# vliu15/3d-brain-tumor-segmentation

Measured on AMD Instinct MI355X. Metric: training volumes/sec (2ch x 128^3), higher is better.
Workload: dtype f32; 1 GPU; BASELINE configs[1]: 2ch x 128^3, batch 1 per GPU, fp32, full fwd+bwd with Dice+KL+L2 VAE loss + Dice metric + TF-form Adam; CLI-default model (base_filters=32, depth=4, groups=8, reduction=8; 42,174,773 params); parallelism=dp1, global_batch=1

## Files before the change

### 3d-brain-tumor-segmentation_amd/csrc/block_bwd.hip

```cpp
#include "common.h"
#include "bts_internal.h"
#include "finalize_parts.h"

__global__ __launch_bounds__(256) void blk_bwd_reduce_kernel(const float* __restrict__ x, const float* __restrict__ dy,
                                                             const float* __restrict__ res, const float* __restrict__ sp,
                                                             const float* __restrict__ gamma, const float* __restrict__ beta,
                                                             const float* __restrict__ mean, const float* __restrict__ rstd,
                                                             double* partial, double* se_partial, float* __restrict__ ds_out, long E, long L,
                                                             long span, int C, int G, int cg, int lddy) {
  __shared__ double sh[256 * 8];
  const int unit = blockIdx.y, n = unit / G, gs = unit % G;
  const long unitBase = (long)gs * L;
  const long lo = (long)blockIdx.x * span;
  long hi = lo + span;
  if (hi > L) hi = L;
  const int F4 = C >> 2;
  const int cph = (int)((unitBase + lo + threadIdx.x * 4) % C);
  float gam[4], bet[4];
#pragma unroll
  for (int e = 0; e < 4; ++e) {
    const int idx = gs * cg + ((cph + e) % cg);
    gam[e] = gamma[idx];
    bet[e] = beta[idx];
  }
  const float m_s = mean[unit], rs_s = rstd[unit];
  double a[4] = {0, 0, 0, 0}, b[4] = {0, 0, 0, 0}, pa[4] = {0, 0, 0, 0}, pb[4] = {0, 0, 0, 0};
  const float* xb = x + (long)n * E + unitBase;
  const float* rb = res + (long)n * E + unitBase;
  const long pix0 = ((long)n * E + unitBase + lo + threadIdx.x * 4) / C;
  const long pstep = 1024 / C;
  const bool head = (threadIdx.x & (F4 - 1)) == 0;
  auto one = [&](const f32x4 v, const f32x4 r, const f32x4 d, float s, long pix) {
    float t = (d[0] * r[0] + d[1] * r[1]) + (d[2] * r[2] + d[3] * r[3]);
    for (int o = F4 >> 1; o > 0; o >>= 1) t += __shfl_xor(t, o, 64);
    const float dsv = t * s * (1.f - s);
    if (head) ds_out[pix] = dsv;
#pragma unroll
    for (int e = 0; e < 4; ++e) {
      const float xh = (v[e] - m_s) * rs_s;
      float de = d[e];
      if (!(xh * gam[e] + bet[e] > 0.f)) de = 0.f;
      a[e] += (double)(de * xh);
      b[e] += (double)de;
      pa[e] += (double)(d[e] * r[e]);
      pb[e] += (double)(dsv * r[e]);
    }
  };
  const long K = (hi - lo) / 1024;
  const long i0 = lo + threadIdx.x * 4;
  long k = 0;
  for (; k + 2 <= K; k += 2) {
    f32x4 v[2], r[2], d[2];
    float s[2];
#pragma unroll
    for (int u = 0; u < 2; ++u) {
      const long i = i0 + (k + u) * 1024, pix = pix0 + (k + u) * pstep;
      v[u] = *reinterpret_cast<const f32x4*>(xb + i);
      r[u] = *reinterpret_cast<const f32x4*>(rb + i);
      d[u] = *reinterpret_cast<const f32x4*>(dy + pix * lddy + cph);
      s[u] = sp[pix];
    }
#pragma unroll
    for (int u = 0; u < 2; ++u) one(v[u], r[u], d[u], s[u], pix0 + (k + u) * pstep);
  }
  for (; k < K; ++k) {
    const long i = i0 + k * 1024, pix = pix0 + k * pstep;
    one(*reinterpret_cast<const f32x4*>(xb + i), *reinterpret_cast<const f32x4*>(rb + i), *reinterpret_cast<const f32x4*>(dy + pix * lddy + cph), sp[pix],
        pix);
  }
#pragma unroll
  for (int e = 0; e < 4; ++e) { sh[threadIdx.x * 8 + e] = a[e]; sh[threadIdx.x * 8 + 4 + e] = b[e]; }
  __syncthreads();
  for (int j = threadIdx.x; j < cg; j += 256) {
    double sa = 0.0, sb = 0.0;
    if (cg >= 4) {
      const int e = j & 3, rr = j >> 2, P4 = cg >> 2;
      for (int q = rr; q < 256; q += P4) { sa += sh[q * 8 + e]; sb += sh[q * 8 + 4 + e]; }
    } else {
      for (int q = 0; q < 256; ++q)
        for (int e = j; e < 4; e += cg) { sa += sh[q * 8 + e]; sb += sh[q * 8 + 4 + e]; }
    }
    const long o = (((long)unit * gridDim.x + blockIdx.x) * cg + j) * 2;
    partial[o] = sa;
    partial[o + 1] = sb;
  }
  __syncthreads();
#pragma unroll
  for (int e = 0; e < 4; ++e) { sh[threadIdx.x * 8 + e] = pa[e]; sh[threadIdx.x * 8 + 4 + e] = pb[e]; }
  __syncthreads();
  const int vpb = 256 / F4;
  for (int col = threadIdx.x; col < C; col += 256) {
    const int e = col & 3, l = col >> 2;
    double sa = 0.0, sb = 0.0;
    for (int q = 0; q < vpb; ++q) { sa += sh[(q * F4 + l) * 8 + e]; sb += sh[(q * F4 + l) * 8 + 4 + e]; }
    const long o = ((((long)n * G + gs) * gridDim.x + blockIdx.x) * C + col) * 2;
    se_partial[o] = sa;
    se_partial[o + 1] = sb;
  }
}

__global__ __launch_bounds__(256) void blk_bwd_apply_kernel(const float* __restrict__ x, const float* __restrict__ dy, float* __restrict__ dx,
                                                            float* __restrict__ dres, const float* __restrict__ gamma,
                                                            const float* __restrict__ beta, const float* __restrict__ mean,
                                                            const float* __restrict__ rstd, const float* __restrict__ c1,
                                                            const float* __restrict__ c2, const float* __restrict__ sp,
                                                            const float* __restrict__ ds, const float* __restrict__ ch,
                                                            const float* __restrict__ wsp, const float* __restrict__ dgap, long chunks_per_unit,
                                                            int cpb, int C, int cg, int G, int lddy) {
  const long chunk0 = (long)blockIdx.x * cpb;
  const long unit = chunk0 / chunks_per_unit;
  const int g = (int)(unit % G), n = (int)(unit / G);
  const float m = mean[unit], rs = rstd[unit], k1 = c1[unit], k2 = c2[unit];
  const int c = (threadIdx.x * 4) % C;
  float ga[4], be[4];
#pragma unroll
  for (int e = 0; e < 4; ++e) {
    const int idx = g * cg + ((c + e) % cg);
    ga[e] = gamma[idx];
    be[e] = beta[idx];
  }
  const f32x4 chv = *reinterpret_cast<const f32x4*>(ch + (long)n * C + c);
  const f32x4 wsv = {wsp[c], wsp[c + 1], wsp[c + 2], wsp[c + 3]};
  const f32x4 dgv = *reinterpret_cast<const f32x4*>(dgap + (long)n * C + c);
  const long off = chunk0 * 1024 + threadIdx.x * 4;
  const long vpc = 1024 / C;
  const long pix = chunk0 * vpc + (threadIdx.x * 4) / C;
  const long doff = pix * lddy + c;
  const long dstep = vpc * lddy;
  auto one = [&](const f32x4 v, const f32x4 d, float s, float dsv, long o_) {
    f32x4 o, q;
#pragma unroll
    for (int e = 0; e < 4; ++e) {
      const float xh = (v[e] - m) * rs;
      float de = d[e];
      if (!(xh * ga[e] + be[e] > 0.f)) de = 0.f;
      o[e] = (de * ga[e] - k1 - xh * k2) * rs;
      q[e] = d[e] * (s + chv[e]) + dsv * wsv[e] + dgv[e];
    }
    *reinterpret_cast<f32x4*>(dx + o_) = o;
    *reinterpret_cast<f32x4*>(dres + o_) = q;
  };
  int k = 0;
  for (; k + 1 < cpb; k += 2) {
    const f32x4 v0 = *reinterpret_cast<const f32x4*>(x + off + (long)k * 1024);
    const f32x4 d0 = *reinterpret_cast<const f32x4*>(dy + doff + (long)k * dstep);
    const f32x4 v1 = *reinterpret_cast<const f32x4*>(x + off + (long)(k + 1) * 1024);
    const f32x4 d1 = *reinterpret_cast<const f32x4*>(dy + doff + (long)(k + 1) * dstep);
    const float s0 = sp[pix + (long)k * vpc], s1 = sp[pix + (long)(k + 1) * vpc];
    const float t0 = ds[pix + (long)k * vpc], t1 = ds[pix + (long)(k + 1) * vpc];
    one(v0, d0, s0, t0, off + (long)k * 1024);
    one(v1, d1, s1, t1, off + (long)(k + 1) * 1024);
  }
  for (; k < cpb; ++k) {
    const f32x4 v0 = *reinterpret_cast<const f32x4*>(x + off + (long)k * 1024);
    const f32x4 d0 = *reinterpret_cast<const f32x4*>(dy + doff + (long)k * dstep);
    one(v0, d0, sp[pix + (long)k * vpc], ds[pix + (long)k * vpc], off + (long)k * 1024);
  }
}

__global__ __launch_bounds__(256) void blk_bwd_middle_kernel(const double* partial, const float* gamma, float* dgamma, float* dbeta, float* c1,
                                                             float* c2, const double* se_partial, double* red, int N, int G, int B, int cg,
                                                             double L, int accum, int F) {
  __shared__ double sh[256 * 2];
  if ((int)blockIdx.x < G) gn_bwd_finalize_slab_body(partial, gamma, dgamma, dbeta, c1, c2, N, G, B, cg, L, accum, blockIdx.x, sh);
  else se_bwd_partial_reduce_body(se_partial, red, N, G * B, F, (int)blockIdx.x - G);
}

static bool blk_bwd_plan(int N, long V, int F, int R, int G, int* B, long* span) {
  if (N <= 0 || V <= 0 || R <= 0 || G <= 0 || F < 4 || F > 256 || (F & (F - 1)) != 0 || F % G != 0) return false;
  const long E = V * F;
  if (E % G != 0) return false;
  const long L = E / G;
  const int cg = F / G;
  if (L % 1024 != 0 || 1024 % F != 0 || 256 % cg != 0) return false;
  if (!bts_gn_slab_blocks_(N, V, F, G, B, span)) return false;
  return (long)N * G * (L / 1024) <= 0x7fffffffL;
}
extern "C" long bts_block_bwd_workspace(int N, long V, int F, int R, int G) {
  int B;
  long span;
  if (!blk_bwd_plan(N, V, F, R, G, &B, &span)) return -1;
  const int cg = F / G;
  return (long)N * G * B * cg * 2 * 8 + (long)N * G * 2 * 4 + 64
         + (long)N * G * B * F * 2 * 8 + ((long)N * F * 3 + (long)N * R) * 8 + 128;
}
extern "C" int bts_block_bwd(const float* dout, int lddo, const float* res, const float* c2x, const float* sp, const float* gap, const float* h,
                             const float* ch, const float* w1, const float* w2, const float* wsp, const float* gamma, const float* beta,
                             const float* mean, const float* rstd, float* dres, float* dc2, float* ds, float* dgap, float* dw1, float* dw2,
                             float* dwsp, float* dgamma, float* dbeta, void* workspace, long workspace_bytes, int N, long V, int F, int R, int G,
                             int accumulate_gate_params, int accumulate_norm_params, hipStream_t stream) {
  int B;
  long span;
  if (!blk_bwd_plan(N, V, F, R, G, &B, &span)) return BTS_ERR_UNSUPPORTED;
  if (lddo < F || lddo % 4 != 0) return BTS_ERR_ALIGN;
  if ((((uintptr_t)dout) & 15) || (((uintptr_t)res) & 15) || (((uintptr_t)c2x) & 15) || (((uintptr_t)dres) & 15) || (((uintptr_t)dc2) & 15) ||
      (((uintptr_t)ch) & 15) || (((uintptr_t)dgap) & 15))
    return BTS_ERR_ALIGN;
  if (workspace == nullptr || (((uintptr_t)workspace) & 15) || workspace_bytes < bts_block_bwd_workspace(N, V, F, R, G)) return BTS_ERR_WORKSPACE;
  const long E = V * F, L = E / G;
  const int cg = F / G;
  double* partial = reinterpret_cast<double*>(workspace);
  float* c1 = reinterpret_cast<float*>(partial + (long)N * G * B * cg * 2);
  float* c2 = c1 + (long)N * G;
  double* sep = reinterpret_cast<double*>((reinterpret_cast<uintptr_t>(c2 + (long)N * G) + 63) & ~(uintptr_t)63);
  double* red = sep + (long)N * G * B * F * 2;
  double* scratch = red + (long)N * F * 2;
  (void)hipGetLastError();
  hipLaunchKernelGGL(blk_bwd_reduce_kernel, dim3(B, N * G), dim3(256), 0, stream, c2x, dout, res, sp, gamma, beta, mean, rstd, partial, sep, ds, E, L,
                     span, F, G, cg, lddo);
  BTS_LAUNCH_CHECK();
  hipLaunchKernelGGL(blk_bwd_middle_kernel, dim3(G + (N * F + 3) / 4), dim3(256), 0, stream, partial, gamma, dgamma, dbeta, c1, c2, sep, red, N, G, B, cg,
                     (double)L, accumulate_norm_params, F);
  BTS_LAUNCH_CHECK();
  const int r = bts_se_mlp_bwd_(red, scratch, gap, h, ch, w1, w2, dw1, dw2, dwsp, dgap, N, G * B, V, F, R, accumulate_gate_params, stream);
  if (r != BTS_OK) return r;
  const long cpu = L / 1024;
  int cpb = 8;
  while (cpb > 1 && cpu % cpb != 0) cpb >>= 1;
  const long nblk = (long)N * G * cpu / cpb;
  hipLaunchKernelGGL(blk_bwd_apply_kernel, dim3((unsigned)nblk), dim3(256), 0, stream, c2x, dout, dc2, dres, gamma, beta, mean, rstd, c1, c2, sp, ds, ch,
                     wsp, dgap, cpu, cpb, F, cg, G, lddo);
  BTS_LAUNCH_CHECK();
  return BTS_OK;
}
```

### 3d-brain-tumor-segmentation_amd/csrc/finalize_parts.h

```cpp
#pragma once
#include "common.h"

__device__ __forceinline__ void gn_bwd_finalize_slab_body(const double* partial, const float* gamma, float* dgamma, float* dbeta, float* c1,
                                                          float* c2, int N, int G, int B, int cg, double L, int accum, int g, double* sh) {
  const int j = threadIdx.x % cg, sl = threadIdx.x / cg, S = 256 / cg;
  double ga = 0.0, gb = 0.0;
  for (int n = 0; n < N; ++n) {
    const long unit = (long)n * G + g;
    double sa = 0.0, sb = 0.0;
    for (int b = sl; b < B; b += S) {
      const double* o = partial + ((unit * B + b) * cg + j) * 2;
      sa += o[0]; sb += o[1];
    }
    __syncthreads();
    sh[threadIdx.x * 2] = sa; sh[threadIdx.x * 2 + 1] = sb;
    __syncthreads();
    if (sl == 0) {
      sa = 0.0; sb = 0.0;
      for (int s2 = 0; s2 < S; ++s2) { sa += sh[(s2 * cg + j) * 2]; sb += sh[(s2 * cg + j) * 2 + 1]; }
      ga += sa; gb += sb;
    }
    __syncthreads();
    if (sl == 0) {
      sh[j * 2] = (double)gamma[g * cg + j] * sb;
      sh[j * 2 + 1] = (double)gamma[g * cg + j] * sa;
    }
    __syncthreads();
    if (threadIdx.x == 0) {
      double s1 = 0.0, s2 = 0.0;
      for (int q = 0; q < cg; ++q) { s1 += sh[q * 2]; s2 += sh[q * 2 + 1]; }
      c1[unit] = (float)(s1 / L);
      c2[unit] = (float)(s2 / L);
    }
  }
  if (sl == 0) {
    const int idx = g * cg + j;
    if (dgamma) dgamma[idx] = accum ? dgamma[idx] + (float)ga : (float)ga;
    if (dbeta) dbeta[idx] = accum ? dbeta[idx] + (float)gb : (float)gb;
  }
}

__device__ __forceinline__ void se_bwd_partial_reduce_body(const double* partial, double* red, int N, int B, int F, int blk) {
  const int lane = threadIdx.x & 63;
  const int i = blk * 4 + (threadIdx.x >> 6);
  if (i >= N * F) return;
  const int n = i / F, c = i % F;
  double a = 0.0, b = 0.0;
  const double2* pp = reinterpret_cast<const double2*>(partial) + (long)n * B * F + c;
  int k = lane;
  for (; k + 7 * 64 < B; k += 8 * 64) {
    double2 v[8];
#pragma unroll
    for (int u = 0; u < 8; ++u) v[u] = pp[(long)(k + u * 64) * F];
#pragma unroll
    for (int u = 0; u < 8; ++u) { a += v[u].x; b += v[u].y; }
  }
  for (; k < B; k += 64) {
    const double2 v = pp[(long)k * F];
    a += v.x;
    b += v.y;
  }
  a = wave_sum_f64(a);
  b = wave_sum_f64(b);
  if (lane == 0) { red[i * 2] = a; red[i * 2 + 1] = b; }
}

__device__ __forceinline__ void se_mlp_bwd_param_body(const double* red, const float* gap, const float* hbuf, float* dw1, float* dw2, float* dwsp,
                                                      const double* scratch, int N, int F, int R, int accum, int blk) {
  const double* dz2 = scratch;
  const double* dz1 = scratch + (long)N * F;
  const int i = blk * 256 + threadIdx.x;
  if (i < R * F) {
    {
      const int k = i / F, c = i % F;
      double s = 0.0;
      for (int n = 0; n < N; ++n) s += (double)hbuf[n * R + k] * dz2[n * F + c];
      dw2[i] = accum ? dw2[i] + (float)s : (float)s;
    }
    {
      const int c = i / R, k = i % R;
      double s = 0.0;
      for (int n = 0; n < N; ++n) s += (double)gap[n * F + c] * dz1[n * R + k];
      dw1[i] = accum ? dw1[i] + (float)s : (float)s;
    }
  }
  if (i < F) {
    double s = 0.0;
    for (int n = 0; n < N; ++n) s += red[((long)n * F + i) * 2 + 1];
    dwsp[i] = accum ? dwsp[i] + (float)s : (float)s;
  }
}

__device__ __forceinline__ void lp_dbias_block(const float (&cs)[8], int oct, int noct, double* part_row, float* sh ) {
  __syncthreads();
#pragma unroll
  for (int e = 0; e < 8; ++e) sh[threadIdx.x * 8 + e] = cs[e];
  __syncthreads();
  if ((int)threadIdx.x < noct * 8) {
    const int o = threadIdx.x >> 3, e = threadIdx.x & 7;
    double s = 0.0;
    for (int t = o; t < 256; t += noct) s += (double)sh[t * 8 + e];
    part_row[o * 8 + e] = s;
  }
  (void)oct;
}
__device__ __forceinline__ void lp_dbias_finalize_body(const double* part, float* db, int nblocks, int C, int accum, int c, double* sh) {
  double s = 0.0;
  for (int b = threadIdx.x; b < nblocks; b += 256) s += part[(long)b * C + c];
  s = block_sum_f64(s, sh);
  if (threadIdx.x == 0) db[c] = accum ? db[c] + (float)s : (float)s;
}

__device__ __forceinline__ void lp_gn_bwd_finalize_body(const double* partial, const float* gamma, float* dgamma, float* dbeta, float* c1,
                                                        float* c2, int N, int G, int B, int cg, double L, int accum, int g, double* sh,
                                                        double* tot ) {
  const int t = threadIdx.x;
  int Np = 1;
  while (Np * 2 <= N && cg * Np * 2 <= 256) Np *= 2;
  const int S = 256 / (cg * Np);
  const int j = t % cg, nl = (t / cg) % Np, sl = t / (cg * Np);
  double ga = 0.0, gb = 0.0;
  for (int n0 = 0; n0 < N; n0 += Np) {
    const int n = n0 + nl;
    double sa = 0.0, sb = 0.0;
    if (n < N) {
      const long unit = (long)n * G + g;
      for (int b = sl; b < B; b += S) {
        const double* o = partial + ((unit * B + b) * cg + j) * 2;
        sa += o[0]; sb += o[1];
      }
    }
    __syncthreads();
    sh[t * 2] = sa; sh[t * 2 + 1] = sb;
    __syncthreads();
    if (sl == 0) {
      sa = 0.0; sb = 0.0;
      for (int s2 = 0; s2 < S; ++s2) { sa += sh[((s2 * Np + nl) * cg + j) * 2]; sb += sh[((s2 * Np + nl) * cg + j) * 2 + 1]; }
      tot[(nl * cg + j) * 2] = sa; tot[(nl * cg + j) * 2 + 1] = sb;
    }
    __syncthreads();
    if (t < Np && n0 + t < N) {
      double s1 = 0.0, s2 = 0.0;
      for (int q = 0; q < cg; ++q) {
        s1 += (double)gamma[g * cg + q] * tot[(t * cg + q) * 2 + 1];
        s2 += (double)gamma[g * cg + q] * tot[(t * cg + q) * 2];
      }
      const long unit = (long)(n0 + t) * G + g;
      c1[unit] = (float)(s1 / L);
      c2[unit] = (float)(s2 / L);
    }
    if (t < cg) {
      for (int q = 0; q < Np && n0 + q < N; ++q) { ga += tot[(q * cg + t) * 2]; gb += tot[(q * cg + t) * 2 + 1]; }
    }
  }
// ... 7 lines not shown
```

### 3d-brain-tumor-segmentation_amd/csrc/groupnorm.hip

```cpp
#include <stdlib.h>
#include "common.h"
#include "bts_internal.h"
#include "finalize_parts.h"

#define GN_BLOCKS_MAX 256

struct GnGeom {
  int N, C, G, cg, mode;
  long V;
  long E;
  long L;
  int B;
  long span;
  int generic;
};

static int gn_geom(GnGeom& g, int N, long V, int C, int G, int mode) {
  if (N <= 0 || V <= 0 || C <= 0 || G <= 0) return BTS_ERR_SHAPE;
  if (C < G || C % G != 0) return BTS_ERR_SHAPE;
  g.N = N; g.C = C; g.G = G; g.cg = C / G; g.mode = mode; g.V = V; g.E = V * C; g.L = g.E / G;
  if (g.E % G != 0) return BTS_ERR_UNSUPPORTED;
  g.generic = (C % 4 != 0 || (C & (C - 1)) != 0 || C > 1024 || g.L % 4 != 0) ? 1 : 0;
  const long unit = (mode == BTS_GN_SLAB) ? g.L : g.E;
  const int units = (mode == BTS_GN_SLAB) ? N * G : N;
// ... 238 lines not shown
  const int lane = threadIdx.x & 63, w = threadIdx.x >> 6;
  if (lane == 0) { sh[w] = s; sh[16 + w] = ss; }
  __syncthreads();
  if (threadIdx.x == 0) {
    double rs = 0.0, rss = 0.0;
    for (int k = 0; k < 16; ++k) { rs += sh[k]; rss += sh[16 + k]; }
    const double m = rs / count;
    double var = rss / count - m * m;
    if (var < 0.0) var = 0.0;
    mean[i] = (float)m;
    rstd[i] = (float)(1.0 / sqrt(var + (double)eps));
  }
}

int bts_gn_finalize_partials_(const double* partial, float* mean, float* rstd, int NG, long B, double count, float eps,
                              hipStream_t stream) {
  if (NG <= 0 || B <= 0 || B > 0x7fffffffL) return BTS_ERR_SHAPE;
  if (B >= 512) {
    if (((uintptr_t)partial) & 15) return BTS_ERR_ALIGN;
    (void)hipGetLastError(); hipLaunchKernelGGL(gn_stats_finalize_wide_kernel, dim3(NG), dim3(1024), 0, stream, partial, mean, rstd, (int)B, count, eps);
    BTS_LAUNCH_CHECK();
    return BTS_OK;
  }
  (void)hipGetLastError(); hipLaunchKernelGGL(gn_stats_finalize_kernel, dim3((NG + 3) / 4), dim3(256), 0, stream, partial, mean, rstd, NG, (int)B, 0,
                     1, BTS_GN_SLAB, count, eps);
  BTS_LAUNCH_CHECK();
  return BTS_OK;
}

__global__ __launch_bounds__(256) void gn_apply_kernel(const float* __restrict__ x, float* __restrict__ y,
                                                       const float* __restrict__ gamma, const float* __restrict__ beta,
                                                       const float* __restrict__ mean, const float* __restrict__ rstd,
                                                       long total4, long E, long L, int C, int G, int cg, int ldy,
                                                       int mode, int relu) {
  for (long f = blockIdx.x * (long)blockDim.x + threadIdx.x; f < total4; f += (long)gridDim.x * blockDim.x) {
    const long i = f * 4;
    const long n = i / E;
    const long r = i - n * E;
    const int c = (int)(r % C);
    const long pix = i / C;
    const f32x4 v = *reinterpret_cast<const f32x4*>(x + i);
    f32x4 o;
    if (mode == BTS_GN_SLAB) {
      const int g = (int)(r / L);
      const float m = mean[n * G + g], rs = rstd[n * G + g];
#pragma unroll
      for (int e = 0; e < 4; ++e) {
        const int idx = g * cg + ((c + e) % cg);
        o[e] = (v[e] - m) * rs * gamma[idx] + beta[idx];
      }
    } else {
#pragma unroll
      for (int e = 0; e < 4; ++e) {
        const int g = (c + e) / cg;
        o[e] = (v[e] - mean[n * G + g]) * rstd[n * G + g] * gamma[c + e] + beta[c + e];
      }
    }
    if (relu) {
#pragma unroll
      for (int e = 0; e < 4; ++e) o[e] = fmaxf(o[e], 0.f);
    }
    *reinterpret_cast<f32x4*>(y + pix * ldy + c) = o;
  }
}

__global__ __launch_bounds__(256) void gn_apply_slab_stream_kernel(const float* __restrict__ x, float* __restrict__ y,
                                                                   const float* __restrict__ gamma, const float* __restrict__ beta,
                                                                   const float* __restrict__ mean, const float* __restrict__ rstd,
                                                                   long chunks_per_unit, int cpb, int C, int cg, int G, int relu, int ldy) {
  const long chunk0 = (long)blockIdx.x * cpb;
  const long unit = chunk0 / chunks_per_unit;
  const int g = (int)(unit % G);
  const float m = mean[unit], rs = rstd[unit];
  const int c = (threadIdx.x * 4) % C;
  float sc[4], sh[4];
#pragma unroll
  for (int e = 0; e < 4; ++e) {
    const int idx = g * cg + ((c + e) % cg);
    sc[e] = rs * gamma[idx];
    sh[e] = beta[idx];
  }
  const float* xp = x + chunk0 * 1024 + threadIdx.x * 4;
  const long vpc = 1024 / C;
  float* yp = y + (chunk0 * vpc + (threadIdx.x * 4) / C) * ldy + c;
  const long ystep = vpc * ldy;
  int k = 0;
  for (; k + 1 < cpb; k += 2) {
    const f32x4 v0 = *reinterpret_cast<const f32x4*>(xp + (long)k * 1024);
    const f32x4 v1 = *reinterpret_cast<const f32x4*>(xp + (long)(k + 1) * 1024);
    f32x4 o0, o1;
#pragma unroll
    for (int e = 0; e < 4; ++e) {
      o0[e] = fmaf(v0[e] - m, sc[e], sh[e]);
      o1[e] = fmaf(v1[e] - m, sc[e], sh[e]);
      if (relu) { o0[e] = fmaxf(o0[e], 0.f); o1[e] = fmaxf(o1[e], 0.f); }
    }
    *reinterpret_cast<f32x4*>(yp + (long)k * ystep) = o0;
    *reinterpret_cast<f32x4*>(yp + (long)(k + 1) * ystep) = o1;
  }
  for (; k < cpb; ++k) {
    const f32x4 v0 = *reinterpret_cast<const f32x4*>(xp + (long)k * 1024);
    f32x4 o0;
#pragma unroll
    for (int e = 0; e < 4; ++e) {
      o0[e] = fmaf(v0[e] - m, sc[e], sh[e]);
      if (relu) o0[e] = fmaxf(o0[e], 0.f);
    }
    *reinterpret_cast<f32x4*>(yp + (long)k * ystep) = o0;
  }
}
static int gn_stream_cpb(long chunks_per_unit) {
  int cpb = 8;
  while (cpb > 1 && chunks_per_unit % cpb != 0) cpb >>= 1;
  return cpb;
}

extern "C" int bts_gn_apply(const float* x, float* y, const float* gamma, const float* beta, const float* mean,
                            const float* rstd, int N, long V, int C, int ldy, int G, int mode, int relu,
                            hipStream_t stream) {
  GnGeom g;
  int r = gn_geom(g, N, V, C, G, mode);
  if (r != BTS_OK) return r;
  if (g.generic || ldy % 4 != 0) {
    if (ldy < C) return BTS_ERR_ALIGN;
    const long total = (long)N * g.E;
    int gb = (int)((total + 255) / 256);
    if (gb > 8192) gb = 8192;
    (void)hipGetLastError(); hipLaunchKernelGGL(gn_apply_generic_kernel, dim3(gb), dim3(256), 0, stream, x, y, gamma, beta, mean, rstd, total, g.E, g.L,
                       C, G, g.cg, ldy, mode, relu);
    BTS_LAUNCH_CHECK();
    return BTS_OK;
  }
  if (ldy < C || (((uintptr_t)x) & 15) || (((uintptr_t)y) & 15)) return BTS_ERR_ALIGN;
  if (mode == BTS_GN_SLAB && g.L % 1024 == 0 && 1024 % C == 0) {
    const long cpu = g.L / 1024;
    const int cpb = gn_stream_cpb(cpu);
    const long nblk = (long)N * G * cpu / cpb;
    if (nblk <= 0x7fffffffL) {
      (void)hipGetLastError(); hipLaunchKernelGGL(gn_apply_slab_stream_kernel, dim3((unsigned)nblk), dim3(256), 0, stream, x, y, gamma, beta, mean,
                         rstd, cpu, cpb, C, g.cg, G, relu, ldy);
      BTS_LAUNCH_CHECK();
      return BTS_OK;
    }
  }
  const long total4 = (long)N * g.E / 4;
  int blocks = (int)((total4 + 255) / 256);
  if (blocks > 8192) blocks = 8192;
  (void)hipGetLastError(); hipLaunchKernelGGL(gn_apply_kernel, dim3(blocks), dim3(256), 0, stream, x, y, gamma, beta, mean, rstd, total4, g.E,
                     g.L, C, G, g.cg, ldy, mode, relu);
  BTS_LAUNCH_CHECK();
  return BTS_OK;
}

__global__ __launch_bounds__(256) void gn_bwd_reduce_kernel(const float* __restrict__ x, const float* __restrict__ dy,
                                                            const float* __restrict__ gamma, const float* __restrict__ beta,
                                                            const float* __restrict__ mean, const float* __restrict__ rstd,
                                                            double* partial, long E, long L, long span, int C, int G,
                                                            int cg, int lddy, int mode, int relu) {
  __shared__ double sh[256 * 8];
  const bool slab = (mode == BTS_GN_SLAB);
  const int n = slab ? blockIdx.y / G : blockIdx.y;
  const int gs = slab ? blockIdx.y % G : 0;
  const long unitBase = slab ? (long)gs * L : 0;
  const long unitLen = slab ? L : E;
  const long lo = (long)blockIdx.x * span;
  long hi = lo + span;
  if (hi > unitLen) hi = unitLen;
  double a[4] = {0, 0, 0, 0}, b[4] = {0, 0, 0, 0};
  const long npix = E / C;
  const int cph = (int)((unitBase + lo + threadIdx.x * 4) % C);
  float gam[4], bet[4];
#pragma unroll
  for (int e = 0; e < 4; ++e) {
    const int idx = slab ? gs * cg + ((cph + e) % cg) : (cph + e);
    gam[e] = gamma[idx];
    bet[e] = beta[idx];
  }
  const float m_s = mean[n * G + gs], rs_s = rstd[n * G + gs];
  auto body = [&](const f32x4 v, const f32x4 d, int c) {
#pragma unroll
    for (int e = 0; e < 4; ++e) {
      const int g = slab ? gs : (c + e) / cg;
      const float xh = slab ? (v[e] - m_s) * rs_s : (v[e] - mean[n * G + g]) * rstd[n * G + g];
      float de = d[e];
      if (relu && !(xh * gam[e] + bet[e] > 0.f)) de = 0.f;
      a[e] += (double)(de * xh);
      b[e] += (double)de;
    }
  };
  long i = lo + threadIdx.x * 4;
  if (lddy == C) {
    const float* xb = x + (long)n * E + unitBase;
    const float* db = dy + (long)n * E + unitBase;
    for (; i + 3072 < hi; i += 4096) {
      f32x4 v[4], d[4];
#pragma unroll
      for (int u = 0; u < 4; ++u) {
        v[u] = *reinterpret_cast<const f32x4*>(xb + i + 1024 * u);
        d[u] = *reinterpret_cast<const f32x4*>(db + i + 1024 * u);
      }
#pragma unroll
      for (int u = 0; u < 4; ++u) body(v[u], d[u], cph);
    }
    for (; i + 1024 < hi; i += 2048) {
      const f32x4 v0 = *reinterpret_cast<const f32x4*>(xb + i);
      const f32x4 v1 = *reinterpret_cast<const f32x4*>(xb + i + 1024);
      const f32x4 d0 = *reinterpret_cast<const f32x4*>(db + i);
      const f32x4 d1 = *reinterpret_cast<const f32x4*>(db + i + 1024);
      body(v0, d0, cph);
      body(v1, d1, cph);
    }
    for (; i < hi; i += 1024) {
      const f32x4 v = *reinterpret_cast<const f32x4*>(xb + i);
      const f32x4 d = *reinterpret_cast<const f32x4*>(db + i);
      body(v, d, cph);
    }
  }
  for (; i + 1024 < hi; i += 2048) {
    const long r0 = unitBase + i, r1 = r0 + 1024;
    const int c0 = (int)(r0 % C), c1 = (int)(r1 % C);
    const f32x4 v0 = *reinterpret_cast<const f32x4*>(x + (long)n * E + r0);
    const f32x4 v1 = *reinterpret_cast<const f32x4*>(x + (long)n * E + r1);
    const f32x4 d0 = *reinterpret_cast<const f32x4*>(dy + ((long)n * npix + r0 / C) * lddy + c0);
    const f32x4 d1 = *reinterpret_cast<const f32x4*>(dy + ((long)n * npix + r1 / C) * lddy + c1);
    body(v0, d0, c0);
    body(v1, d1, c1);
  }
  for (; i < hi; i += 1024) {
    const long r = unitBase + i;
    const int c = (int)(r % C);
    const f32x4 v = *reinterpret_cast<const f32x4*>(x + (long)n * E + r);
    const f32x4 d = *reinterpret_cast<const f32x4*>(dy + ((long)n * npix + r / C) * lddy + c);
    body(v, d, c);
  }
#pragma unroll
  for (int e = 0; e < 4; ++e) { sh[threadIdx.x * 8 + e] = a[e]; sh[threadIdx.x * 8 + 4 + e] = b[e]; }
  __syncthreads();
  const int P = slab ? cg : C;
  for (int j = threadIdx.x; j < P; j += 256) {
    double sa = 0.0, sb = 0.0;
    if (P >= 4) {
      const int e = j & 3, rr = j >> 2, P4 = P >> 2;
      for (int k = rr; k < 256; k += P4) { sa += sh[k * 8 + e]; sb += sh[k * 8 + 4 + e]; }
    } else {
      for (int k = 0; k < 256; ++k)
        for (int e = j; e < 4; e += P) { sa += sh[k * 8 + e]; sb += sh[k * 8 + 4 + e]; }
    }
    const long o = (((long)blockIdx.y * gridDim.x + blockIdx.x) * P + j) * 2;
    partial[o] = sa;
    partial[o + 1] = sb;
  }
}

__global__ __launch_bounds__(256) void gn_bwd_finalize_a_kernel(const double* partial, double* scratch, int N, int B, int C,
                                                                int G, int mode) {
  const int lane = threadIdx.x & 63;
  const int t = blockIdx.x * 4 + (threadIdx.x >> 6);
  if (t >= N * C) return;
  const int cg = C / G;
  const int n = t / C, idx = t % C;
  double sa = 0.0, sb = 0.0;
  if (mode == BTS_GN_SLAB) {
    const int g = idx / cg, j = idx % cg;
    for (int b = lane; b < B; b += 64) {
      const long o = ((((long)n * G + g) * B + b) * cg + j) * 2;
      sa += partial[o];
      sb += partial[o + 1];
    }
  } else {
    for (int b = lane; b < B; b += 64) {
      const long o = (((long)n * B + b) * C + idx) * 2;
      sa += partial[o];
      sb += partial[o + 1];
    }
  }
  sa = wave_sum_f64(sa);
  sb = wave_sum_f64(sb);
  if (lane == 0) { scratch[t * 2] = sa; scratch[t * 2 + 1] = sb; }
}
__global__ void gn_bwd_finalize_kernel(const float* gamma, float* dgamma, float* dbeta, float* c1, float* c2,
                                       const double* scratch , int N, int C, int G, double L, int accum) {
  const int cg = C / G;
  for (int idx = threadIdx.x; idx < C; idx += blockDim.x) {
    double sa = 0.0, sb = 0.0;
    for (int n = 0; n < N; ++n) { sa += scratch[(n * C + idx) * 2]; sb += scratch[(n * C + idx) * 2 + 1]; }
    if (dgamma) dgamma[idx] = accum ? dgamma[idx] + (float)sa : (float)sa;
    if (dbeta) dbeta[idx] = accum ? dbeta[idx] + (float)sb : (float)sb;
  }
  for (int t = threadIdx.x; t < N * G; t += blockDim.x) {
    const int n = t / G, g = t % G;
    double s1 = 0.0, s2 = 0.0;
    for (int j = 0; j < cg; ++j) {
      const int idx = g * cg + j;
      s1 += (double)gamma[idx] * scratch[(n * C + idx) * 2 + 1];
      s2 += (double)gamma[idx] * scratch[(n * C + idx) * 2];
    }
    c1[t] = (float)(s1 / L);
    c2[t] = (float)(s2 / L);
  }
}

__global__ __launch_bounds__(256) void gn_bwd_finalize_slab_kernel(const double* partial, const float* gamma, float* dgamma, float* dbeta, float* c1,
                                                                   float* c2, int N, int G, int B, int cg, double L, int accum) {
  __shared__ double sh[256 * 2];
  gn_bwd_finalize_slab_body(partial, gamma, dgamma, dbeta, c1, c2, N, G, B, cg, L, accum, blockIdx.x, sh);
}

__global__ __launch_bounds__(256) void gn_bwd_apply_kernel(const float* __restrict__ x, const float* __restrict__ dy,
                                                           float* __restrict__ dx, const float* __restrict__ gamma,
                                                           const float* __restrict__ beta, const float* __restrict__ mean,
                                                           const float* __restrict__ rstd, const float* __restrict__ c1,
                                                           const float* __restrict__ c2, long total4, long E, long L,
                                                           int C, int G, int cg, int lddy, int mode, int relu) {
  const long f0 = blockIdx.x * (long)blockDim.x + threadIdx.x;
  const int cph = (int)((f0 * 4) % C);
  const bool fixed = ((long)gridDim.x * 1024) % C == 0;
  for (long f = f0; f < total4; f += (long)gridDim.x * blockDim.x) {
    const long i = f * 4;
    const long n = i / E;
    const long r = i - n * E;
    const int c = fixed ? cph : (int)(r % C);
    const long pix = i / C;
    const f32x4 v = *reinterpret_cast<const f32x4*>(x + i);
    const f32x4 d = *reinterpret_cast<const f32x4*>(dy + pix * lddy + c);
    const int gsl = (int)(r / L);
    f32x4 o;
#pragma unroll
    for (int e = 0; e < 4; ++e) {
      const int g = (mode == BTS_GN_SLAB) ? gsl : (c + e) / cg;
      const int idx = (mode == BTS_GN_SLAB) ? g * cg + ((c + e) % cg) : (c + e);
      const float rs = rstd[n * G + g];
      const float xh = (v[e] - mean[n * G + g]) * rs;
      float de = d[e];
      const float ga = gamma[idx];
      if (relu && !(xh * ga + beta[idx] > 0.f)) de = 0.f;
      o[e] = (de * ga - c1[n * G + g] - xh * c2[n * G + g]) * rs;
    }
    *reinterpret_cast<f32x4*>(dx + i) = o;
  }
}

bool bts_gn_slab_blocks_(int N, long V, int C, int G, int* B, long* span) {
  GnGeom g;
  if (gn_geom(g, N, V, C, G, BTS_GN_SLAB) != BTS_OK || g.generic) return false;
  *B = g.B;
  *span = g.span;
  return true;
}
__global__ __launch_bounds__(256) void gn_bwd_apply_slab_stream_kernel(const float* __restrict__ x, const float* __restrict__ dy,
                                                                       float* __restrict__ dx, const float* __restrict__ gamma,
                                                                       const float* __restrict__ beta, const float* __restrict__ mean,
                                                                       const float* __restrict__ rstd, const float* __restrict__ c1,
                                                                       const float* __restrict__ c2, long chunks_per_unit, int cpb,
                                                                       int C, int cg, int G, int relu, int lddy) {
  const long chunk0 = (long)blockIdx.x * cpb;
  const long unit = chunk0 / chunks_per_unit;
  const int g = (int)(unit % G);
  const float m = mean[unit], rs = rstd[unit], k1 = c1[unit], k2 = c2[unit];
  const int c = (threadIdx.x * 4) % C;
  float ga[4], be[4];
#pragma unroll
  for (int e = 0; e < 4; ++e) {
    const int idx = g * cg + ((c + e) % cg);
    ga[e] = gamma[idx];
    be[e] = beta[idx];
  }
  const long off = chunk0 * 1024 + threadIdx.x * 4;
  const long vpc = 1024 / C;
  const long doff = (chunk0 * vpc + (threadIdx.x * 4) / C) * lddy + c;
  const long dstep = vpc * lddy;
  auto one = [&](const f32x4 v, const f32x4 d) {
    f32x4 o;
#pragma unroll
    for (int e = 0; e < 4; ++e) {
      const float xh = (v[e] - m) * rs;
      float de = d[e];
      if (relu && !(xh * ga[e] + be[e] > 0.f)) de = 0.f;
      o[e] = (de * ga[e] - k1 - xh * k2) * rs;
    }
    return o;
  };
  int k = 0;
  for (; k + 1 < cpb; k += 2) {
    const f32x4 v0 = *reinterpret_cast<const f32x4*>(x + off + (long)k * 1024);
    const f32x4 d0 = *reinterpret_cast<const f32x4*>(dy + doff + (long)k * dstep);
    const f32x4 v1 = *reinterpret_cast<const f32x4*>(x + off + (long)(k + 1) * 1024);
    const f32x4 d1 = *reinterpret_cast<const f32x4*>(dy + doff + (long)(k + 1) * dstep);
    *reinterpret_cast<f32x4*>(dx + off + (long)k * 1024) = one(v0, d0);
    *reinterpret_cast<f32x4*>(dx + off + (long)(k + 1) * 1024) = one(v1, d1);
  }
  for (; k < cpb; ++k) {
    const f32x4 v0 = *reinterpret_cast<const f32x4*>(x + off + (long)k * 1024);
    const f32x4 d0 = *reinterpret_cast<const f32x4*>(dy + doff + (long)k * dstep);
    *reinterpret_cast<f32x4*>(dx + off + (long)k * 1024) = one(v0, d0);
  }
}

extern "C" int bts_gn_bwd(const float* x, const float* dy, float* dx, const float* gamma, const float* beta,
                          const float* mean, const float* rstd, float* dgamma, float* dbeta, void* workspace,
                          long workspace_bytes, int N, long V, int C, int lddy, int G, int mode, int relu,
                          int accumulate_params, hipStream_t stream) {
  GnGeom g;
  int r = gn_geom(g, N, V, C, G, mode);
  if (r != BTS_OK) return r;
  if (lddy < C) return BTS_ERR_ALIGN;
  if (workspace == nullptr) return BTS_ERR_WORKSPACE;
  if (g.generic || lddy % 4 != 0) {
    if (workspace_bytes < (long)N * G * 2 * 4 + 64) return BTS_ERR_WORKSPACE;
    float* gc1 = reinterpret_cast<float*>(workspace);
    float* gc2 = gc1 + (long)N * G;
    (void)hipGetLastError(); hipLaunchKernelGGL(gn_bwd_group_generic_kernel, dim3(N * G), dim3(256), 0, stream, x, dy, gamma, beta, mean, rstd, gc1, gc2,
                       g.E, g.L, C, G, g.cg, lddy, mode, relu);
    BTS_LAUNCH_CHECK();
    (void)hipGetLastError(); hipLaunchKernelGGL(gn_bwd_param_generic_kernel, dim3(C), dim3(256), 0, stream, x, dy, gamma, beta, mean, rstd, dgamma, dbeta,
                       N, g.E, g.L, C, G, g.cg, lddy, mode, relu, accumulate_params);
    BTS_LAUNCH_CHECK();
    const long total = (long)N * g.E;
    int gb = (int)((total + 255) / 256);
    if (gb > 8192) gb = 8192;
    (void)hipGetLastError(); hipLaunchKernelGGL(gn_bwd_apply_generic_kernel, dim3(gb), dim3(256), 0, stream, x, dy, dx, gamma, beta, mean, rstd, gc1, gc2,
                       total, g.E, g.L, C, G, g.cg, lddy, mode, relu);
    BTS_LAUNCH_CHECK();
    return BTS_OK;
  }
  if ((((uintptr_t)x) & 15) || (((uintptr_t)dy) & 15) || (((uintptr_t)dx) & 15)) return BTS_ERR_ALIGN;
  const long part_bytes = bts_gn_workspace(N, V, C, G, mode);
  const long extra = (long)N * C * 2 * 8 + (long)N * G * 2 * 4 + 64;
  if (workspace_bytes < part_bytes + extra) return BTS_ERR_WORKSPACE;
  double* partial = reinterpret_cast<double*>(workspace);
  double* scratch = reinterpret_cast<double*>(reinterpret_cast<char*>(workspace) + ((part_bytes + 15) & ~15L));
  float* c1 = reinterpret_cast<float*>(scratch + (long)N * C * 2);
  float* c2 = c1 + (long)N * G;
  const bool slab = (mode == BTS_GN_SLAB);
  (void)hipGetLastError(); hipLaunchKernelGGL(gn_bwd_reduce_kernel, dim3(g.B, slab ? N * G : N), dim3(256), 0, stream, x, dy, gamma, beta, mean,
                     rstd, partial, g.E, g.L, g.span, C, G, g.cg, lddy, mode, relu);
  BTS_LAUNCH_CHECK();
  if (slab && g.cg <= 256 && 256 % g.cg == 0) {
    (void)hipGetLastError(); hipLaunchKernelGGL(gn_bwd_finalize_slab_kernel, dim3(G), dim3(256), 0, stream, partial, gamma, dgamma, dbeta, c1, c2, N, G, g.B,
                       g.cg, (double)g.L, accumulate_params);
    BTS_LAUNCH_CHECK();
  } else {
    (void)hipGetLastError(); hipLaunchKernelGGL(gn_bwd_finalize_a_kernel, dim3((N * C + 3) / 4), dim3(256), 0, stream, partial, scratch, N, g.B, C, G, mode);
    BTS_LAUNCH_CHECK();
    (void)hipGetLastError(); hipLaunchKernelGGL(gn_bwd_finalize_kernel, dim3(1), dim3(256), 0, stream, gamma, dgamma, dbeta, c1, c2, scratch, N, C, G,
                       (double)g.L, accumulate_params);
    BTS_LAUNCH_CHECK();
  }
  if (slab && g.L % 1024 == 0 && 1024 % C == 0) {
    const long cpu = g.L / 1024;
    const int cpb = gn_stream_cpb(cpu);
    const long nblk = (long)N * G * cpu / cpb;
    if (nblk <= 0x7fffffffL) {
      (void)hipGetLastError(); hipLaunchKernelGGL(gn_bwd_apply_slab_stream_kernel, dim3((unsigned)nblk), dim3(256), 0, stream, x, dy, dx, gamma, beta,
                         mean, rstd, c1, c2, cpu, cpb, C, g.cg, G, relu, lddy);
      BTS_LAUNCH_CHECK();
      return BTS_OK;
    }
  }
  const long total4 = (long)N * g.E / 4;
  int blocks = (int)((total4 + 255) / 256);
  if (blocks > 8192) blocks = 8192;
  (void)hipGetLastError(); hipLaunchKernelGGL(gn_bwd_apply_kernel, dim3(blocks), dim3(256), 0, stream, x, dy, dx, gamma, beta, mean, rstd, c1, c2,
                     total4, g.E, g.L, C, G, g.cg, lddy, mode, relu);
  BTS_LAUNCH_CHECK();
  return BTS_OK;
}

extern "C" long bts_gn_bwd_workspace(int N, long V, int C, int G, int mode) {
  const long p = bts_gn_workspace(N, V, C, G, mode);
  if (p < 0) return -1;
  return ((p + 15) & ~15L) + (long)N * C * 2 * 8 + (long)N * G * 2 * 4 + 64;
}
```

Before: 29.19 volumes/s.

## Interleave GroupNorm backward reduce chunks across blocks and pre-fold shared partials

Both backward reduce kernels (the fused block one and the generic GroupNorm one) now give each block interleaved 1024-element chunks (k, k+B, …) instead of one contiguous span. This drops the span argument and spreads adjacent memory across concurrently running blocks. A new `fold_rows_f64` helper first folds the 256 per-thread double partials into 32 rows in shared memory when the channel period allows, shortening the serial per-column summation tail. The generic reduce kernel is also templated on slab/relu and given a launch-bounds occupancy hint of 5, at the cost of more instantiations and possible register pressure.

```diff
diff --git a/3d-brain-tumor-segmentation_amd/csrc/block_bwd.hip b/3d-brain-tumor-segmentation_amd/csrc/block_bwd.hip
--- a/3d-brain-tumor-segmentation_amd/csrc/block_bwd.hip
+++ b/3d-brain-tumor-segmentation_amd/csrc/block_bwd.hip
@@ -7,15 +7,14 @@
                                                              const float* __restrict__ gamma, const float* __restrict__ beta,
                                                              const float* __restrict__ mean, const float* __restrict__ rstd,
                                                              double* partial, double* se_partial, float* __restrict__ ds_out, long E, long L,
-                                                             long span, int C, int G, int cg, int lddy) {
+                                                             int C, int G, int cg, int lddy) {
   __shared__ double sh[256 * 8];
+  __shared__ double rows[32 * 8];
   const int unit = blockIdx.y, n = unit / G, gs = unit % G;
   const long unitBase = (long)gs * L;
-  const long lo = (long)blockIdx.x * span;
-  long hi = lo + span;
-  if (hi > L) hi = L;
+  const long t4 = threadIdx.x * 4;
   const int F4 = C >> 2;
-  const int cph = (int)((unitBase + lo + threadIdx.x * 4) % C);
+  const int cph = (int)((unitBase + t4) % C);
   float gam[4], bet[4];
 #pragma unroll
   for (int e = 0; e < 4; ++e) {
@@ -27,7 +26,7 @@
   double a[4] = {0, 0, 0, 0}, b[4] = {0, 0, 0, 0}, pa[4] = {0, 0, 0, 0}, pb[4] = {0, 0, 0, 0};
   const float* xb = x + (long)n * E + unitBase;
   const float* rb = res + (long)n * E + unitBase;
-  const long pix0 = ((long)n * E + unitBase + lo + threadIdx.x * 4) / C;
+  const long pix0 = ((long)n * E + unitBase + t4) / C;
   const long pstep = 1024 / C;
   const bool head = (threadIdx.x & (F4 - 1)) == 0;
   auto one = [&](const f32x4 v, const f32x4 r, const f32x4 d, float s, long pix) {
@@ -46,39 +45,46 @@
       pb[e] += (double)(dsv * r[e]);
     }
   };
-  const long K = (hi - lo) / 1024;
-  const long i0 = lo + threadIdx.x * 4;
-  long k = 0;
-  for (; k + 2 <= K; k += 2) {
+  const long K = L >> 10, B = gridDim.x;
+  auto trip1 = [&](long k) {
+    const long i = k * 1024 + t4, pix = pix0 + k * pstep;
+    one(*reinterpret_cast<const f32x4*>(xb + i), *reinterpret_cast<const f32x4*>(rb + i), *reinterpret_cast<const f32x4*>(dy + pix * lddy + cph), sp[pix],
+        pix);
+  };
+  long k = blockIdx.x;
+  for (; k + B < K; k += 2 * B) {
     f32x4 v[2], r[2], d[2];
     float s[2];
 #pragma unroll
     for (int u = 0; u < 2; ++u) {
-      const long i = i0 + (k + u) * 1024, pix = pix0 + (k + u) * pstep;
+      const long i = (k + u * B) * 1024 + t4, pix = pix0 + (k + u * B) * pstep;
       v[u] = *reinterpret_cast<const f32x4*>(xb + i);
       r[u] = *reinterpret_cast<const f32x4*>(rb + i);
       d[u] = *reinterpret_cast<const f32x4*>(dy + pix * lddy + cph);
       s[u] = sp[pix];
     }
 #pragma unroll
-    for (int u = 0; u < 2; ++u) one(v[u], r[u], d[u], s[u], pix0 + (k + u) * pstep);
-  }
-  for (; k < K; ++k) {
-    const long i = i0 + k * 1024, pix = pix0 + k * pstep;
-    one(*reinterpret_cast<const f32x4*>(xb + i), *reinterpret_cast<const f32x4*>(rb + i), *reinterpret_cast<const f32x4*>(dy + pix * lddy + cph), sp[pix],
-        pix);
-  }
+    for (int u = 0; u < 2; ++u) one(v[u], r[u], d[u], s[u], pix0 + (k + u * B) * pstep);
+  }
+  if (k < K) trip1(k);
 #pragma unroll
   for (int e = 0; e < 4; ++e) { sh[threadIdx.x * 8 + e] = a[e]; sh[threadIdx.x * 8 + 4 + e] = b[e]; }
   __syncthreads();
+  const double* src = sh;
+  int nrows = 256;
+  if (cg <= 128) {
+    fold_rows_f64(sh, rows);
+    src = rows;
+    nrows = 32;
+  }
   for (int j = threadIdx.x; j < cg; j += 256) {
     double sa = 0.0, sb = 0.0;
     if (cg >= 4) {
       const int e = j & 3, rr = j >> 2, P4 = cg >> 2;
-      for (int q = rr; q < 256; q += P4) { sa += sh[q * 8 + e]; sb += sh[q * 8 + 4 + e]; }
+      for (int q = rr; q < nrows; q += P4) { sa += src[q * 8 + e]; sb += src[q * 8 + 4 + e]; }
     } else {
-      for (int q = 0; q < 256; ++q)
-        for (int e = j; e < 4; e += cg) { sa += sh[q * 8 + e]; sb += sh[q * 8 + 4 + e]; }
+      for (int q = 0; q < nrows; ++q)
+        for (int e = j; e < 4; e += cg) { sa += src[q * 8 + e]; sb += src[q * 8 + 4 + e]; }
     }
     const long o = (((long)unit * gridDim.x + blockIdx.x) * cg + j) * 2;
     partial[o] = sa;
@@ -88,11 +94,17 @@
 #pragma unroll
   for (int e = 0; e < 4; ++e) { sh[threadIdx.x * 8 + e] = pa[e]; sh[threadIdx.x * 8 + 4 + e] = pb[e]; }
   __syncthreads();
-  const int vpb = 256 / F4;
+  src = sh;
+  nrows = 256;
+  if (F4 <= 32) {
+    fold_rows_f64(sh, rows);
+    src = rows;
+    nrows = 32;
+  }
   for (int col = threadIdx.x; col < C; col += 256) {
     const int e = col & 3, l = col >> 2;
     double sa = 0.0, sb = 0.0;
-    for (int q = 0; q < vpb; ++q) { sa += sh[(q * F4 + l) * 8 + e]; sb += sh[(q * F4 + l) * 8 + 4 + e]; }
+    for (int q = l; q < nrows; q += F4) { sa += src[q * 8 + e]; sb += src[q * 8 + 4 + e]; }
     const long o = ((((long)n * G + gs) * gridDim.x + blockIdx.x) * C + col) * 2;
     se_partial[o] = sa;
     se_partial[o + 1] = sb;
@@ -207,7 +219,7 @@
   double* scratch = red + (long)N * F * 2;
   (void)hipGetLastError();
   hipLaunchKernelGGL(blk_bwd_reduce_kernel, dim3(B, N * G), dim3(256), 0, stream, c2x, dout, res, sp, gamma, beta, mean, rstd, partial, sep, ds, E, L,
-                     span, F, G, cg, lddo);
+                     F, G, cg, lddo);
   BTS_LAUNCH_CHECK();
   hipLaunchKernelGGL(blk_bwd_middle_kernel, dim3(G + (N * F + 3) / 4), dim3(256), 0, stream, partial, gamma, dgamma, dbeta, c1, c2, sep, red, N, G, B, cg,
                      (double)L, accumulate_norm_params, F);
diff --git a/3d-brain-tumor-segmentation_amd/csrc/finalize_parts.h b/3d-brain-tumor-segmentation_amd/csrc/finalize_parts.h
--- a/3d-brain-tumor-segmentation_amd/csrc/finalize_parts.h
+++ b/3d-brain-tumor-segmentation_amd/csrc/finalize_parts.h
@@ -1,5 +1,13 @@
 #pragma once
 #include "common.h"
+
+__device__ __forceinline__ void fold_rows_f64(const double* sh , double* rows ) {
+  double s = 0.0;
+#pragma unroll
+  for (int k = 0; k < 8; ++k) s += sh[threadIdx.x + 256 * k];
+  rows[threadIdx.x] = s;
+  __syncthreads();
+}
 
 __device__ __forceinline__ void gn_bwd_finalize_slab_body(const double* partial, const float* gamma, float* dgamma, float* dbeta, float* c1,
                                                           float* c2, int N, int G, int B, int cg, double L, int accum, int g, double* sh) {
diff --git a/3d-brain-tumor-segmentation_amd/csrc/groupnorm.hip b/3d-brain-tumor-segmentation_amd/csrc/groupnorm.hip
--- a/3d-brain-tumor-segmentation_amd/csrc/groupnorm.hip
+++ b/3d-brain-tumor-segmentation_amd/csrc/groupnorm.hip
@@ -414,23 +414,24 @@
   return BTS_OK;
 }
 
-__global__ __launch_bounds__(256) void gn_bwd_reduce_kernel(const float* __restrict__ x, const float* __restrict__ dy,
-                                                            const float* __restrict__ gamma, const float* __restrict__ beta,
-                                                            const float* __restrict__ mean, const float* __restrict__ rstd,
-                                                            double* partial, long E, long L, long span, int C, int G,
-                                                            int cg, int lddy, int mode, int relu) {
+template <bool slab, bool relu>
+__global__ __launch_bounds__(256, 5) void gn_bwd_reduce_kernel(const float* __restrict__ x, const float* __restrict__ dy,
+                                                               const float* __restrict__ gamma, const float* __restrict__ beta,
+                                                               const float* __restrict__ mean, const float* __restrict__ rstd,
+                                                               double* partial, long E, long L, int C, int G, int cg, int lddy) {
   __shared__ double sh[256 * 8];
-  const bool slab = (mode == BTS_GN_SLAB);
+  __shared__ double rows[32 * 8];
   const int n = slab ? blockIdx.y / G : blockIdx.y;
   const int gs = slab ? blockIdx.y % G : 0;
   const long unitBase = slab ? (long)gs * L : 0;
   const long unitLen = slab ? L : E;
-  const long lo = (long)blockIdx.x * span;
-  long hi = lo + span;
-  if (hi > unitLen) hi = unitLen;
+  const long nfull = unitLen >> 10;
+  const long B = gridDim.x;
+  const unsigned t4u = threadIdx.x * 4;
+  const long t4 = t4u;
   double a[4] = {0, 0, 0, 0}, b[4] = {0, 0, 0, 0};
   const long npix = E / C;
-  const int cph = (int)((unitBase + lo + threadIdx.x * 4) % C);
+  const int cph = (int)((unitBase + t4) % C);
   float gam[4], bet[4];
 #pragma unroll
   for (int e = 0; e < 4; ++e) {
@@ -450,63 +451,62 @@
       b[e] += (double)de;
     }
   };
-  long i = lo + threadIdx.x * 4;
+  const float* xb = x + (long)n * E + unitBase;
+  long k = blockIdx.x;
   if (lddy == C) {
-    const float* xb = x + (long)n * E + unitBase;
     const float* db = dy + (long)n * E + unitBase;
-    for (; i + 3072 < hi; i += 4096) {
+    for (; k + 3 * B < nfull; k += 4 * B) {
       f32x4 v[4], d[4];
 #pragma unroll
       for (int u = 0; u < 4; ++u) {
-        v[u] = *reinterpret_cast<const f32x4*>(xb + i + 1024 * u);
-        d[u] = *reinterpret_cast<const f32x4*>(db + i + 1024 * u);
+        v[u] = *reinterpret_cast<const f32x4*>(xb + (k + u * B) * 1024 + t4u);
+        d[u] = *reinterpret_cast<const f32x4*>(db + (k + u * B) * 1024 + t4u);
       }
 #pragma unroll
       for (int u = 0; u < 4; ++u) body(v[u], d[u], cph);
     }
-    for (; i + 1024 < hi; i += 2048) {
-      const f32x4 v0 = *reinterpret_cast<const f32x4*>(xb + i);
-      const f32x4 v1 = *reinterpret_cast<const f32x4*>(xb + i + 1024);
-      const f32x4 d0 = *reinterpret_cast<const f32x4*>(db + i);
-      const f32x4 d1 = *reinterpret_cast<const f32x4*>(db + i + 1024);
+    for (; k * 1024 < unitLen; k += B) {
+      const long i = k * 1024 + t4;
+      if (i < unitLen) body(*reinterpret_cast<const f32x4*>(xb + i), *reinterpret_cast<const f32x4*>(db + i), cph);
+    }
+  } else {
+    auto dptr = [&](long i) {
+      const long r = unitBase + i;
+      return dy + ((long)n * npix + r / C) * lddy + (int)(r % C);
+    };
+    for (; k + B < nfull; k += 2 * B) {
+      const long i0 = k * 1024 + t4, i1 = (k + B) * 1024 + t4;
+      const f32x4 v0 = *reinterpret_cast<const f32x4*>(xb + i0);
+      const f32x4 v1 = *reinterpret_cast<const f32x4*>(xb + i1);
+      const f32x4 d0 = *reinterpret_cast<const f32x4*>(dptr(i0));
+      const f32x4 d1 = *reinterpret_cast<const f32x4*>(dptr(i1));
       body(v0, d0, cph);
       body(v1, d1, cph);
     }
-    for (; i < hi; i += 1024) {
-      const f32x4 v = *reinterpret_cast<const f32x4*>(xb + i);
-      const f32x4 d = *reinterpret_cast<const f32x4*>(db + i);
-      body(v, d, cph);
-    }
-  }
-  for (; i + 1024 < hi; i += 2048) {
-    const long r0 = unitBase + i, r1 = r0 + 1024;
-    const int c0 = (int)(r0 % C), c1 = (int)(r1 % C);
-    const f32x4 v0 = *reinterpret_cast<const f32x4*>(x + (long)n * E + r0);
-    const f32x4 v1 = *reinterpret_cast<const f32x4*>(x + (long)n * E + r1);
-    const f32x4 d0 = *reinterpret_cast<const f32x4*>(dy + ((long)n * npix + r0 / C) * lddy + c0);
-    const f32x4 d1 = *reinterpret_cast<const f32x4*>(dy + ((long)n * npix + r1 / C) * lddy + c1);
-    body(v0, d0, c0);
-    body(v1, d1, c1);
-  }
-  for (; i < hi; i += 1024) {
-    const long r = unitBase + i;
-    const int c = (int)(r % C);
-    const f32x4 v = *reinterpret_cast<const f32x4*>(x + (long)n * E + r);
-    const f32x4 d = *reinterpret_cast<const f32x4*>(dy + ((long)n * npix + r / C) * lddy + c);
-    body(v, d, c);
+    for (; k * 1024 < unitLen; k += B) {
+      const long i = k * 1024 + t4;
+      if (i < unitLen) body(*reinterpret_cast<const f32x4*>(xb + i), *reinterpret_cast<const f32x4*>(dptr(i)), cph);
+    }
   }
 #pragma unroll
   for (int e = 0; e < 4; ++e) { sh[threadIdx.x * 8 + e] = a[e]; sh[threadIdx.x * 8 + 4 + e] = b[e]; }
   __syncthreads();
   const int P = slab ? cg : C;
+  const double* src = sh;
+  int nrows = 256;
+  if (P <= 128) {
+    fold_rows_f64(sh, rows);
+    src = rows;
+    nrows = 32;
+  }
   for (int j = threadIdx.x; j < P; j += 256) {
     double sa = 0.0, sb = 0.0;
     if (P >= 4) {
       const int e = j & 3, rr = j >> 2, P4 = P >> 2;
-      for (int k = rr; k < 256; k += P4) { sa += sh[k * 8 + e]; sb += sh[k * 8 + 4 + e]; }
+      for (int q = rr; q < nrows; q += P4) { sa += src[q * 8 + e]; sb += src[q * 8 + 4 + e]; }
     } else {
-      for (int k = 0; k < 256; ++k)
-        for (int e = j; e < 4; e += P) { sa += sh[k * 8 + e]; sb += sh[k * 8 + 4 + e]; }
+      for (int q = 0; q < nrows; ++q)
+        for (int e = j; e < 4; e += P) { sa += src[q * 8 + e]; sb += src[q * 8 + 4 + e]; }
     }
     const long o = (((long)blockIdx.y * gridDim.x + blockIdx.x) * P + j) * 2;
     partial[o] = sa;
@@ -694,8 +694,12 @@
   float* c1 = reinterpret_cast<float*>(scratch + (long)N * C * 2);
   float* c2 = c1 + (long)N * G;
   const bool slab = (mode == BTS_GN_SLAB);
-  (void)hipGetLastError(); hipLaunchKernelGGL(gn_bwd_reduce_kernel, dim3(g.B, slab ? N * G : N), dim3(256), 0, stream, x, dy, gamma, beta, mean,
-                     rstd, partial, g.E, g.L, g.span, C, G, g.cg, lddy, mode, relu);
+  (void)hipGetLastError();
+#define GN_BWD_REDUCE(S, R) hipLaunchKernelGGL((gn_bwd_reduce_kernel<S, R>), dim3(g.B, S ? N * G : N), dim3(256), 0, stream, x, dy, gamma, beta, mean, \
+                                               rstd, partial, g.E, g.L, C, G, g.cg, lddy)
+  if (slab) { if (relu) GN_BWD_REDUCE(true, true); else GN_BWD_REDUCE(true, false); }
+  else { if (relu) GN_BWD_REDUCE(false, true); else GN_BWD_REDUCE(false, false); }
+#undef GN_BWD_REDUCE
   BTS_LAUNCH_CHECK();
   if (slab && g.cg <= 256 && 256 % g.cg == 0) {
     (void)hipGetLastError(); hipLaunchKernelGGL(gn_bwd_finalize_slab_kernel, dim3(G), dim3(256), 0, stream, partial, gamma, dgamma, dbeta, c1, c2, N, G, g.B,
```

Measured after the change: 29.40 volumes/s, median of 6. About the same (+0.7%).
